# DIVE128/DMVSNet

Measured on AMD Instinct MI355X. Metric: depth-maps/sec, DTU 1600x1184 5-view 3-stage (64/32/8 hyp), higher is better.
Workload: dtype f32; 1 GPU; BASELINE configs[1]: 1600x1184, 5 views, 64/32/8 hypotheses, 3 stage(s) x (main + 4-plane refine); parallelism=1 GPU, k1=warp_corr_q4 (quad-planar features, one launch configuration per shape), conv_backend=auto, streams=2, maps_in_flight=1, hip_graph=False

## Files before the change

### dmvsnet_amd/csrc/conv3d_mfma.hip

```cpp
#ifndef DMVS_KO
#define DMVS_KO 0
#endif
#ifndef DMVS_X
#define DMVS_X 0
#endif
#include "common.h"
#include "tile_loader.h"

#include <algorithm>
#include <cstdlib>
#include <mutex>


#include <map>
#include <type_traits>
#include <utility>

int dmvs_ensure_dynamic_lds(const void* kernel, size_t lds_bytes) {
    static std::mutex mu;
    static std::map<std::pair<int, const void*>, size_t> configured;
    int dev = 0;
    if (hipGetDevice(&dev) != hipSuccess) return (int)hipGetLastError();
    std::lock_guard<std::mutex> lock(mu);
    auto key = std::make_pair(dev, kernel);
    auto it = configured.find(key);
    if (it == configured.end() || it->second < lds_bytes) {
        hipError_t e = hipFuncSetAttribute(kernel, hipFuncAttributeMaxDynamicSharedMemorySize, (int)lds_bytes);
        if (e != hipSuccess) return (int)e;
        configured[key] = lds_bytes;
    }
    return 0;
}

long g_single_buf_min_blocks = 0;
long g_min_blocks = 768, g_split_blocks = 1024;
long g_deconv_prefetch = 1;

#ifdef DMVS_K3_TRACE
__device__ unsigned long long* g_k3_trace;
extern "C" int dmvs_dev_trace_k3(void* p) { return (int)hipMemcpyToSymbol(HIP_SYMBOL(g_k3_trace), &p, sizeof(p)); }
#define K3_NOW() __builtin_amdgcn_s_memtime()
#define K3_TR(slot, val) do { if (threadIdx.x == 0 && g_k3_trace && blockIdx.x < 65536) g_k3_trace[(size_t)blockIdx.x * 16 + (slot)] = (val); } while (0)
#define K3_TR_HW() do { if (threadIdx.x == 0 && g_k3_trace && blockIdx.x < 65536) { unsigned hw, xcc; asm volatile("s_getreg_b32 %0, hwreg(HW_REG_HW_ID)" : "=s"(hw)); \
    asm volatile("s_getreg_b32 %0, hwreg(HW_REG_XCC_ID)" : "=s"(xcc)); g_k3_trace[(size_t)blockIdx.x * 16 + 15] = hw; g_k3_trace[(size_t)blockIdx.x * 16 + 14] = xcc; } } while (0)
#else
#define K3_NOW() 0ull
#define K3_TR(slot, val) do { } while (0)
#define K3_TR_HW() do { } while (0)
#endif

namespace {

struct ConvArgs {
    const float* in;
    float* out;
    const float* w;
    const float* scale;
    const float* shift;
    const float* skip;
    int Cin, Cout, D, H, W, Do, Ho, Wo, relu;
    int skip_up2;
    int nx, ny, nz;
    int st4;
    int in_cs, in_zs, in_elems;
    int single_buf;
    int outq4;
};

typedef float acc16_t __attribute__((ext_vector_type(16)));
typedef float acc4_t __attribute__((ext_vector_type(4)));

template <int M> struct Frag;
template <> struct Frag<32> {
    static constexpr int KK = 2, NV = 32, ACC = 16;
    typedef acc16_t acc_t;
    static __device__ __forceinline__ acc_t mfma(float a, float b, acc_t c) {
        return __builtin_amdgcn_mfma_f32_32x32x2f32(a, b, c, 0, 0, 0);
    }
    static __device__ __forceinline__ int row(int r, int lk) { return (r & 3) + 8 * (r >> 2) + 4 * lk; }
};
template <> struct Frag<16> {
    static constexpr int KK = 4, NV = 16, ACC = 4;
    typedef acc4_t acc_t;
    static __device__ __forceinline__ acc_t mfma(float a, float b, acc_t c) {
        return __builtin_amdgcn_mfma_f32_16x16x4f32(a, b, c, 0, 0, 0);
    }
    static __device__ __forceinline__ int row(int r, int lk) { return lk * 4 + r; }
};

// ... 308 lines not shown
                    : (rok && ox < a.Wo) ? (unsigned)((oz * (a.Ho >> 1) + (oy >> 1)) * (a.Wo >> 1) + (ox >> 1)) * 4u : kInvalid;
                float sk[F::ACC];
#pragma unroll
                for (int rr = 0; rr < F::ACC; ++rr) {
                    const unsigned so = a.skip_up2 ? cooff[rr] >> 2 : cooff[rr];
                    sk[rr] = (DMVS_KO & 4) ? 0.f : __builtin_bit_cast(float, __builtin_amdgcn_raw_buffer_load_b32(rs_skip, ((spos | cooff[rr]) & kInvalid) ? kInvalid : spos + so, 0, 0));
                }
                if (a.outq4) {
                    typedef unsigned v4u_t __attribute__((ext_vector_type(4)));
                    const int ch = a.Cout >> 1, cq = ch >> 2;
#pragma unroll
                    for (int q = 0; q < F::ACC / 4; ++q) {
                        const int co0 = (mb0 + mb) * M + F::row(4 * q, lk), hsel = co0 >= ch ? 1 : 0;
                        float w4[4];
#pragma unroll
                        for (int e = 0; e < 4; ++e) w4[e] = fmaxf(acc[mb][i][xb][4 * q + e] * sc[4 * q + e] + sh[4 * q + e], lo) + sk[4 * q + e];
                        const unsigned off = (!(pos & kInvalid) && co0 < a.Cout)
                            ? (unsigned)(((hsel * a.Do + oz) * cq + ((co0 - hsel * ch) >> 2)) * out_plane + oy * a.Wo + ox) * 16u : kInvalid;
                        v4u_t qv;
                        qv.x = __builtin_bit_cast(unsigned, w4[0]); qv.y = __builtin_bit_cast(unsigned, w4[1]);
                        qv.z = __builtin_bit_cast(unsigned, w4[2]); qv.w = __builtin_bit_cast(unsigned, w4[3]);
                        __builtin_amdgcn_raw_buffer_store_b128(qv, rs_out, off, 0, 0);
                    }
                } else
#pragma unroll
                for (int rr = 0; rr < F::ACC; ++rr) {
                    const unsigned off = (pos | cooff[rr]) & kInvalid ? kInvalid : pos + cooff[rr];
                    const float v = fmaxf(acc[mb][i][xb][rr] * sc[rr] + sh[rr], lo) + sk[rr];
                    if ((DMVS_KO & 4) && v != 1234.56789f) continue;
                    __builtin_amdgcn_raw_buffer_store_b32(__builtin_bit_cast(unsigned, v), rs_out, off, 0, 0);
                }
            }
        }
    }
    }
#ifdef DMVS_K3_TRACE
    asm volatile("s_waitcnt vmcnt(0)" ::: "memory");
    K3_TR(4, K3_NOW());
#endif
}

template <int M, int KD, int CI_CH, int TZ, int TY, bool PYM = false, int NMB = 1>
struct DeconvGeom {
    static constexpr int IZ = KD == 3 ? TZ + 1 : TZ, IY = TY + 1, IX = 33, IXP = 34;
    static constexpr int PS = IZ * IY * IXP;
    static constexpr int GPC = CI_CH / Frag<M>::KK;
    static constexpr int TILE_F = (CI_CH * PS + 63) & ~63;
    static constexpr int WROWS = (PYM ? (KD == 3 ? 18 : 6) : (KD == 3 ? 27 : 9)) * GPC * NMB;
    static constexpr int BUF_F = TILE_F + WROWS * 64;
};

template <int M, int KD, int CI_CH, int TZ, int TY, bool PYM, bool PREF, int NCH = 0, int NMB = 1, bool ZSKIP = false>
__global__ __launch_bounds__(256, (M == 16 ? 3 : 1)) void deconv_mfma_kernel(ConvArgs a) {
    static_assert(!ZSKIP || (KD == 3 && TZ == 1), "the flat tile of a 3x3x3 layer");
    typedef Frag<M> F;
    typedef typename F::acc_t acc_t;
    typedef DeconvGeom<M, KD, CI_CH, TZ, TY, PYM, NMB> G;
    static_assert(NMB == 1 || (NMB == 2 && M == 16 && !PYM && !PREF), "M-block split: two 16-channel blocks");
    static_assert(!PYM || M == 16, "y-parity merge is the Cout = 8 layout of the 16-row MFMA");
    constexpr int NPY = PYM ? 1 : 2;
    constexpr int XB = 32 / F::NV;
    constexpr int NPZ = KD == 3 ? 2 : 1;
    constexpr int IZ = G::IZ, IY = G::IY, IX = G::IX, IXP = G::IXP, PS = G::PS, GPC = G::GPC;
    constexpr int WROWS = G::WROWS, BUF_F = G::BUF_F;
    static_assert(TZ * TY * NMB == 4, "one (input row, M block) per wave");
    extern __shared__ __attribute__((aligned(16))) float smem[];

    const int tid = threadIdx.x, lane = tid & 63;
    const int wave = __builtin_amdgcn_readfirstlane(tid >> 6);
    const int ln = lane % F::NV, lk = lane / F::NV;
    const int rwave = NMB == 2 ? (wave >> 1) : wave, mb = NMB == 2 ? (wave & 1) : 0;
    const int tz = rwave / TY, ty = rwave % TY;
    int bx, by, bz;
    if (!xcd_tile(a.nx, a.ny, a.nz, KD == 3, bx, by, bz)) return;
    const int ix0 = bx * 32, iy0 = by * TY, iz0 = bz * TZ;

    acc_t acc[NPZ][NPY][2][XB];
#pragma unroll
    for (int pz = 0; pz < NPZ; ++pz)
#pragma unroll
        for (int p = 0; p < 2 * NPY; ++p)
#pragma unroll
            for (int xb = 0; xb < XB; ++xb)
#pragma unroll
                for (int r = 0; r < F::ACC; ++r) acc[pz][p >> 1][p & 1][xb][r] = 0.f;

    const int in_vol = a.D * a.H * a.W;
    auto chunk_rsrc = [&](int ci0, int nch) {
        return __builtin_amdgcn_make_buffer_rsrc((void*)(a.in + (size_t)ci0 * in_vol), (short)0, nch * in_vol * 4, 0x00020000);
    };
    const int nchunks = PREF ? NCH : a.Cin / CI_CH;
    const __amdgpu_buffer_rsrc_t rs_w =
        __builtin_amdgcn_make_buffer_rsrc((void*)a.w, (short)0, nchunks * WROWS * 256, 0x00020000);

    constexpr unsigned kInvalid = 0x80000000u;
    constexpr int NGRP = XB * NPZ * NPY;
    const int out_plane = a.Ho * a.Wo, out_vol = a.Do * out_plane;
    const bool has_skip = a.skip != nullptr;
    const char* skp = reinterpret_cast<const char*>(has_skip ? a.skip : a.out);
    float2_t skv[PREF ? NGRP : 1][F::ACC];
    auto group_pos = [&](int g) -> unsigned {
        const int xb = g / (NPZ * NPY), pz = (g / NPY) % NPZ, pyi = g % NPY;
        const int iz = iz0 + tz, iy = iy0 + ty, ix = ix0 + xb * F::NV + ln;
        const bool ok = iz < a.D && iy < a.H && ix < a.W;
        const int py = PYM ? (lk >> 1) : pyi;
        const int oz = KD == 3 ? 2 * iz + pz : iz;
        return ok ? (unsigned)(oz * out_plane + (2 * iy + py) * a.Wo + 2 * ix) * 4u : kInvalid;
    };
    auto chan_off = [&](int rr) -> unsigned {
        const int co = PYM ? (F::row(rr, lk) & 7) : mb * M + F::row(rr, lk);
        return co < a.Cout ? (unsigned)(co * out_vol) * 4u : kInvalid;
    };
    auto prefetch_group = [&](auto g_t) {
        constexpr int g = decltype(g_t)::value;
        if constexpr (PREF) {
            const unsigned pos = group_pos(g);
#pragma unroll
            for (int rr = 0; rr < F::ACC; ++rr) {
                const unsigned co = chan_off(rr);
                const bool inr = !((pos | co) & kInvalid) && has_skip;
                skv[g][rr] = *reinterpret_cast<const float2_t*>(skp + (inr ? (pos + co) : 0u));
            }
        }
    };
    auto prefetch_at = [&](int c) {
        if constexpr (PREF) {
            asm volatile("" ::: "memory");
            static_assert(NGRP <= 8, "prefetch groups");
#define DMVS_PF(G_) if constexpr (G_ < NGRP) { if (c == 0) prefetch_group(std::integral_constant<int, G_>{}); }
            DMVS_PF(0) DMVS_PF(1) DMVS_PF(2) DMVS_PF(3) DMVS_PF(4) DMVS_PF(5) DMVS_PF(6) DMVS_PF(7)
#undef DMVS_PF
            asm volatile("" ::: "memory");
        }
    };

    float sc[F::ACC], sh[F::ACC];
    unsigned cooff[F::ACC];
    auto load_bn = [&]() {
#pragma unroll
    for (int rr = 0; rr < F::ACC; ++rr) {
        const int co = PYM ? (F::row(rr, lk) & 7) : mb * M + F::row(rr, lk);
        const bool cok = co < a.Cout;
        const int coc = cok ? co : 0;
        if (M == 32 && a.Cout == 32 && (DMVS_X & 2)) {
            const int c0 = F::row(rr, 0);
            const float s0 = a.scale ? a.scale[c0] : 1.f, s1 = a.scale ? a.scale[c0 + 4] : 1.f;
            const float h0 = a.scale ? a.shift[c0] : 0.f, h1 = a.scale ? a.shift[c0 + 4] : 0.f;
            sc[rr] = lk ? s1 : s0;
            sh[rr] = lk ? h1 : h0;
        } else {
            sc[rr] = a.scale ? a.scale[coc] : 1.f;
            sh[rr] = a.scale ? a.shift[coc] : 0.f;
        }
        cooff[rr] = cok ? (unsigned)(co * out_vol) * 4u : kInvalid;
    }
    };
    constexpr bool BN_FIRST = PREF || !(DMVS_X & 4);
    if constexpr (BN_FIRST) load_bn();
    if constexpr (PREF) asm volatile("" ::: "memory");
    K3_TR(0, K3_NOW());
    K3_TR_HW();
    [[maybe_unused]] unsigned long long tr_wait = 0, tr_mfma = 0, tr_t = K3_NOW();
    load_tile<CI_CH, IZ, IY, IX, IXP, PS, false>(a.D, a.H, a.W, chunk_rsrc(0, CI_CH), smem, 0, iz0, iy0, ix0, wave, lane);
    load_weights<WROWS>(rs_w, smem + G::TILE_F, 0, wave, lane);
#pragma unroll(PREF ? NCH : 1)
    for (int c = 0; c < (PREF ? NCH : nchunks); ++c) {
        if (PREF && c == 1) {
            static_assert(!PREF || NGRP * F::ACC == 16, "counted wait of the prefetch");
            asm volatile("s_waitcnt vmcnt(16)" ::: "memory");
        } else {
            asm volatile("s_waitcnt vmcnt(0)" ::: "memory");
        }
        __syncthreads();
#ifdef DMVS_K3_TRACE
        { const unsigned long long n = K3_NOW(); tr_wait += n - tr_t; tr_t = n; if (c == 0) K3_TR(1, n); }
#endif
        float* cur = smem + (c & 1) * BUF_F;
        if (c + 1 < nchunks) {
            float* nxt = smem + ((c + 1) & 1) * BUF_F;
            load_tile<CI_CH, IZ, IY, IX, IXP, PS, false>(a.D, a.H, a.W, chunk_rsrc((c + 1) * CI_CH, CI_CH), nxt, (c + 1) * CI_CH, iz0, iy0, ix0, wave, lane);
            load_weights<WROWS>(rs_w, nxt + G::TILE_F, c + 1, wave, lane);
        }
        prefetch_at(c);
        const float* tile = cur;
        const float* wl = cur + G::TILE_F + lane;
        int step = 0;
#pragma unroll
        for (int oz = 0; oz < NPZ; ++oz)
#pragma unroll
            for (int oy = 0; oy < 2; ++oy)
#pragma unroll
                for (int ox = 0; ox < 2; ++ox)
#pragma unroll
                    for (int g = 0; g < GPC; ++g) {
                        if (ZSKIP && oz == 1) continue;
                        float bv[XB];
#pragma unroll
                        for (int xb = 0; xb < XB; ++xb)
                            bv[xb] = tile[(g * F::KK + lk) * PS + ((tz + oz) * IY + ty + oy) * IXP + xb * F::NV + ln + ox];
#pragma unroll
                        for (int pz = oz; pz < NPZ; ++pz)
#pragma unroll
                            for (int py = PYM ? 0 : oy; py < NPY; ++py)
#pragma unroll
                                for (int px = ox; px < 2; ++px) {
                                    const float av = wl[(step * NMB + mb) * 64];
                                    ++step;
#pragma unroll
                                    for (int xb = 0; xb < XB; ++xb)
                                        acc[pz][py][px][xb] = F::mfma(av, bv[xb], acc[pz][py][px][xb]);
                                }
                    }
#ifdef DMVS_K3_TRACE
        { asm volatile("s_nop 0" ::: "memory"); const unsigned long long n = K3_NOW(); tr_mfma += n - tr_t; tr_t = n; }
#endif
    }
    K3_TR(2, K3_NOW());
    K3_TR(8, tr_wait);
    K3_TR(9, tr_mfma);

    typedef unsigned v2u_t __attribute__((ext_vector_type(2)));
    const int iz = iz0 + tz, iy = iy0 + ty;
    const bool rok = iz < a.D && iy < a.H;
    const __amdgpu_buffer_rsrc_t rs_out =
        __builtin_amdgcn_make_buffer_rsrc((void*)a.out, (short)0, a.Cout * out_vol * 4, 0x00020000);
    const float lo = a.relu ? 0.f : -INFINITY;
    if constexpr (!BN_FIRST) load_bn();
#pragma unroll
    for (int xb = 0; xb < XB; ++xb) {
        const int ix = ix0 + xb * F::NV + ln;
        const bool ok = rok && ix < a.W;
#pragma unroll
        for (int pz = 0; pz < NPZ; ++pz)
#pragma unroll
            for (int pyi = 0; pyi < NPY; ++pyi) {
                const int py = PYM ? (lk >> 1) : pyi;
                const int oz = KD == 3 ? 2 * iz + pz : iz;
                const unsigned pos = ok ? (unsigned)(oz * out_plane + (2 * iy + py) * a.Wo + 2 * ix) * 4u : kInvalid;
                float2_t sk[F::ACC];
#pragma unroll
                for (int rr = 0; rr < F::ACC; ++rr) {
                    const bool inr = !((pos | cooff[rr]) & kInvalid) && has_skip;
                    float2_t t;
                    if constexpr (PREF) t = skv[(xb * NPZ + pz) * NPY + pyi][rr];
                    else t = *reinterpret_cast<const float2_t*>(skp + (inr ? (pos + cooff[rr]) : 0u));
                    sk[rr].x = inr ? t.x : 0.f;
                    sk[rr].y = inr ? t.y : 0.f;
                }
#pragma unroll
                for (int rr = 0; rr < F::ACC; ++rr) {
                    const unsigned off = (pos | cooff[rr]) & kInvalid ? kInvalid : pos + cooff[rr];
                    const float vx = fmaxf(acc[pz][pyi][0][xb][rr] * sc[rr] + sh[rr], lo) + sk[rr].x;
                    const float vy = fmaxf(acc[pz][pyi][1][xb][rr] * sc[rr] + sh[rr], lo) + sk[rr].y;
                    v2u_t v;
                    v.x = __builtin_bit_cast(unsigned, vx);
                    v.y = __builtin_bit_cast(unsigned, vy);
                    __builtin_amdgcn_raw_buffer_store_b64(v, rs_out, off, 0, 0);
                }
            }
    }
#ifdef DMVS_K3_TRACE
    K3_TR(3, K3_NOW());
    asm volatile("s_waitcnt vmcnt(0)" ::: "memory");
    K3_TR(4, K3_NOW());
#endif
}

#ifndef DMVS_CONV1_CI
#define DMVS_CONV1_CI 1
#endif
constexpr int CI_CONV1 = DMVS_CONV1_CI;
#include "dev_guard.h"
constexpr int CI_CONV2 = 4, CI_CONV4 = 2, CI_CONV6 = 4, CI_CONV6_2D = 4;
constexpr int CI_F00 = 2, CI_F01 = 4, CI_F1 = 4, CI_F2 = 4, CI_FO3 = 4, CI_K5A = 2, CI_K5B = 2;
constexpr int CI_K1 = 4;
constexpr int DCI11 = 4, DCI9 = 4;
struct Cfg { int cin, cout, mode, kd, M, MB, ci_ch, pym; };
const Cfg kCfgs[] = {
    {2, 16, DMVS_CONV_S1, 3, 16, 1, 2},
    {8, 16, DMVS_CONV_S2, 3, 16, 1, CI_CONV1},
    {16, 16, DMVS_CONV_S1, 3, 16, 1, CI_CONV2},
    {16, 32, DMVS_CONV_S2, 3, 32, 1, 2},
    {32, 32, DMVS_CONV_S1, 3, 32, 1, CI_CONV4},
    {32, 64, DMVS_CONV_S2, 3, 32, 2, 2},
    {64, 64, DMVS_CONV_S1, 3, 32, 2, CI_CONV6},
    {64, 32, DMVS_DECONV_S2, 3, 16, 2, 8},
    {32, 16, DMVS_DECONV_S2, 3, 16, 1, DCI9},
    {16, 8, DMVS_DECONV_S2, 3, 16, 1, DCI11, 1},
    {32, 64, DMVS_CONV_S2, 1, 32, 2, 2},
    {64, 64, DMVS_CONV_S1, 1, 32, 2, CI_CONV6_2D},
    {64, 32, DMVS_DECONV_S2, 1, 16, 2, 8},
    {4, 8, DMVS_CONV_S1, 1, 16, 1, CI_F00},
    {8, 8, DMVS_CONV_S1, 1, 16, 1, CI_F01},
    {8, 16, DMVS_CONV2D_K5S2, 1, 16, 1, CI_K5A},
    {16, 16, DMVS_CONV_S1, 1, 16, 1, CI_F1},
    {16, 32, DMVS_CONV2D_K5S2, 1, 32, 1, CI_K5B},
    {32, 32, DMVS_CONV_S1, 1, 32, 1, CI_F2},
    {32, 16, DMVS_CONV_S1, 1, 16, 1, CI_FO3},
    {32, 64, DMVS_CONV2D_K1, 1, 32, 2, CI_K1},
    {16, 32, DMVS_CONV2D_K1, 1, 32, 1, CI_K1},
    {8, 32, DMVS_CONV2D_K1, 1, 32, 1, CI_K1},
    {16, 32, DMVS_CONV_S1, 1, 32, 1, 4},
    {64, 32, DMVS_CONV2D_K1, 1, 32, 1, CI_K1},
    {32, 16, DMVS_CONV2D_K1, 1, 16, 1, CI_K1},
    {32, 8, DMVS_CONV2D_K1, 1, 16, 1, CI_K1},
};

int taps_of(int mode, int kdepth) {
    return mode == DMVS_CONV2D_K5S2 ? 25 : mode == DMVS_CONV2D_K1 ? 1 : 9 * kdepth;
}

const Cfg* find_cfg(int cin, int cout, int mode, int kdepth) {
    for (const Cfg& c : kCfgs)
        if (c.cin == cin && c.cout == cout && c.mode == mode && c.kd == kdepth) return &c;
    return nullptr;
}

int tap_of(int p, int o) { return p == 0 ? 1 : (o == 0 ? 2 : 0); }
// ... 29 lines not shown

template <int M, int MB, int STRIDE, int KD, int KS, int CI_CH, int TZ, int TY, bool MBS = false>
int launch_conv_tile(const ConvArgs& a, hipStream_t st) {
    return can_v4(a) ? launch_conv_tile_v<M, MB, STRIDE, KD, KS, CI_CH, TZ, TY, true, MBS>(a, st)
                     : launch_conv_tile_v<M, MB, STRIDE, KD, KS, CI_CH, TZ, TY, false, MBS>(a, st);
}

#define kSplitBlocks g_split_blocks
constexpr int kPlanMBS = 1 << 17;
inline int conv_tile_choice(int stride, int kd, int Do, int Ho, int Wo, int MB) {
    const bool flat = (kd == 1) || Do == 1;
    const int big_ty_flat = (stride == 1) ? 16 : 8, big_ty = (stride == 1) ? 8 : 4;
    const long big_blocks = flat ? (long)ceil_div(Wo, 32) * ceil_div(Ho, big_ty_flat) * Do
                                 : (long)ceil_div(Wo, 32) * ceil_div(Ho, big_ty) * ceil_div(Do, 2);
    const bool big = big_blocks >= kMinBlocks;
    if (!big && MB == 2) {
        const long small_blocks = flat ? (long)ceil_div(Wo, 32) * ceil_div(Ho, 4) * Do
                                       : (long)ceil_div(Wo, 32) * ceil_div(Ho, 2) * ceil_div(Do, 2);
        if (small_blocks < kSplitBlocks) return kPlanMBS | (flat ? 256 + 2 : 2 * 256 + 1);
    }
    if (flat) return 256 + (big ? big_ty_flat : 4);
    return 2 * 256 + (big ? big_ty : 2);
}

template <int M, int MB, int STRIDE, int KD, int CI_CH, int KS = 3>
int launch_conv(const ConvArgs& a, hipStream_t st) {
    constexpr int BIG_TY_FLAT = (STRIDE == 1) ? 16 : 8, BIG_TY = (STRIDE == 1) ? 8 : 4;
    const int choice = conv_tile_choice(STRIDE, KD, a.Do, a.Ho, a.Wo, MB);
    const int tz = (choice >> 8) & 255, ty = choice & 255;
    if constexpr (MB == 2) {
        if (choice & kPlanMBS) {
            if (tz == 1) return launch_conv_tile<M, MB, STRIDE, KD, KS, CI_CH, 1, 2, true>(a, st);
            if (KD == 3) return launch_conv_tile<M, MB, STRIDE, 3, 3, CI_CH, 2, 1, true>(a, st);
            return DMVS_EUNSUPPORTED;
        }
    }
    if (tz == 1) {
        if (ty == BIG_TY_FLAT) return launch_conv_tile<M, MB, STRIDE, KD, KS, CI_CH, 1, BIG_TY_FLAT>(a, st);
        return launch_conv_tile<M, MB, STRIDE, KD, KS, CI_CH, 1, 4>(a, st);
    }
    if (KD == 3) {
        if (ty == BIG_TY) return launch_conv_tile<M, MB, STRIDE, 3, 3, CI_CH, 2, BIG_TY>(a, st);
        return launch_conv_tile<M, MB, STRIDE, 3, 3, CI_CH, 2, 2>(a, st);
    }
    return DMVS_EUNSUPPORTED;
}

template <int M, int KD, int CI_CH, int TZ, int TY, bool PYM, int NMB = 1>
int launch_deconv_tile(const ConvArgs& a, hipStream_t st) {
    typedef DeconvGeom<M, KD, CI_CH, TZ, TY, PYM, NMB> G;
    constexpr size_t lds = 2 * (size_t)G::BUF_F * sizeof(float);
    static_assert(lds <= 160 * 1024, "two pipeline stages must fit the 160 KB LDS");
    dim3 grid(ceil_div(a.W, 32), ceil_div(a.H, TY), ceil_div(a.D, TZ));
    const bool zskip = KD == 3 && TZ == 1 && zpad_skip_wanted(a.D) && a.D == 1 && !(zpad_live_mask(DMVS_ZFORM_T2, a.D, 0, 1) & 1u);
    if constexpr (PYM)
        if (a.skip && g_deconv_prefetch && a.Cin == 4 * CI_CH) {
            if constexpr (KD == 3 && TZ == 1)
                if (zskip) return launch_with_lds(deconv_mfma_kernel<M, KD, CI_CH, TZ, TY, PYM, true, 4, 1, true>, grid, lds, a, st);
            return launch_with_lds(deconv_mfma_kernel<M, KD, CI_CH, TZ, TY, PYM, true, 4>, grid, lds, a, st);
        }
    if constexpr (KD == 3 && TZ == 1)
        if (zskip) return launch_with_lds(deconv_mfma_kernel<M, KD, CI_CH, TZ, TY, PYM, false, 0, NMB, true>, grid, lds, a, st);
    return launch_with_lds(deconv_mfma_kernel<M, KD, CI_CH, TZ, TY, PYM, false, 0, NMB>, grid, lds, a, st);
}

template <int M, int KD, int CI_CH, bool PYM = false, int NMB = 1>
int launch_deconv(const ConvArgs& a, hipStream_t st) {
    if constexpr (NMB == 2) {
        if (KD == 1 || a.D == 1) return launch_deconv_tile<M, KD, CI_CH, 1, 2, PYM, 2>(a, st);
        return launch_deconv_tile<M, 3, CI_CH, 2, 1, PYM, 2>(a, st);
    } else {
        if (KD == 1 || a.D == 1) return launch_deconv_tile<M, KD, CI_CH, 1, 4, PYM>(a, st);
        return launch_deconv_tile<M, 3, CI_CH, 2, 2, PYM>(a, st);
    }
}

}

extern "C" long dmvs_conv3d_mfma_weight_floats(int Cin, int Cout, int mode, int kdepth) {
    const Cfg* c = find_cfg(Cin, Cout, mode, kdepth);
    if (!c) return 0;
    const int KK = c->M == 32 ? 2 : 4, nt = taps_of(mode, kdepth);
    if (c->ci_ch < KK) {
        const int tpg = KK / c->ci_ch;
        return (long)(Cin / c->ci_ch) * ((nt + tpg - 1) / tpg) * c->MB * 64;
    }
    if (c->pym) return (long)(nt / 3 * 2) * (Cin / KK) * 64;
    return (long)nt * (Cin / KK) * c->MB * 64;
}

extern "C" int dmvs_pack_conv_weights_mfma(const float* w, float* out, int Cin, int Cout, int mode, int kdepth) {
    const Cfg* c = find_cfg(Cin, Cout, mode, kdepth);
    if (!c || !w || !out) return DMVS_EUNSUPPORTED;
    const int M = c->M, KK = (M == 32 ? 2 : 4), GPC = c->ci_ch / KK, NT = taps_of(mode, kdepth);
    size_t n = 0;
    for (int ci0 = 0; ci0 < Cin; ci0 += c->ci_ch) {
        if (mode != DMVS_DECONV_S2 && c->ci_ch < KK) {
            const int tpg = KK / c->ci_ch, nsteps = (NT + tpg - 1) / tpg;
            for (int st = 0; st < nsteps; ++st)
                for (int mb = 0; mb < c->MB; ++mb)
                    for (int l = 0; l < 64; ++l) {
                        const int co = mb * M + l % M, k = l / M, ci = ci0 + k % c->ci_ch, t = st * tpg + k / c->ci_ch;
                        out[n++] = (co < Cout && t < NT) ? w[((size_t)co * Cin + ci) * NT + t] : 0.f;
                    }
        } else if (mode != DMVS_DECONV_S2) {
            for (int t = 0; t < NT; ++t)
                for (int g = 0; g < GPC; ++g)
                    for (int mb = 0; mb < c->MB; ++mb)
                        for (int l = 0; l < 64; ++l) {
                            const int co = mb * M + l % M, ci = ci0 + g * KK + l / M;
                            out[n++] = co < Cout ? w[((size_t)co * Cin + ci) * NT + t] : 0.f;
                        }
        } else {
            const int npz = kdepth == 3 ? 2 : 1;
            for (int oz = 0; oz < npz; ++oz)
                for (int oy = 0; oy < 2; ++oy)
// ... 101 lines not shown
```

### dmvsnet_amd/csrc/layout.hip

```cpp
#include "common.h"

#include <cstring>

template <int C>
__global__ __launch_bounds__(256) void nchw_to_hwc_kernel(const float* __restrict__ src, long chan_stride, int c0, int HW,
                                                          float* __restrict__ dst) {
    __shared__ float tile[C * 257];
    const int p0 = blockIdx.x * 256;
    const int t = threadIdx.x;
    const int np = min(256, HW - p0);
    if (t < np) {
#pragma unroll
        for (int c = 0; c < C; ++c) tile[c * 257 + t] = src[(size_t)(c0 + c) * chan_stride + p0 + t];
    }
    __syncthreads();
    const int total = np * C;
    float* out = dst + (size_t)p0 * C;
#pragma unroll
    for (int k = 0; k < C; ++k) {
        const int i = k * 256 + t;
        if (i < total) out[i] = tile[(i % C) * 257 + (i / C)];
    }
}

// ... 246 lines not shown
        return;
    }
    float sy = ((float)y + 0.5f) * 0.5f - 0.5f; sy = sy < 0.f ? 0.f : sy;
    float sx = ((float)x + 0.5f) * 0.5f - 0.5f; sx = sx < 0.f ? 0.f : sx;
    const int y0 = (int)sy, x0 = (int)sx;
    const int y1 = min(y0 + 1, h - 1), x1 = min(x0 + 1, w - 1);
    const float ly = sy - (float)y0, lx = sx - (float)x0;
    const float hy = 1.f - ly, hx = 1.f - lx;
    const float l00 = last[y0 * w + x0], l01 = last[y0 * w + x1], l10 = last[y1 * w + x0], l11 = last[y1 * w + x1];
    const bool s00 = ((y0 & 1) == (x0 & 1)), s01 = ((y0 & 1) == (x1 & 1));
    const bool s10 = ((y1 & 1) == (x0 & 1)), s11 = ((y1 & 1) == (x1 & 1));
    for (int d = 0; d < nplanes; ++d) {
        const float v00 = hyp_sample(l00, s00, pix, D, d, inverse), v01 = hyp_sample(l01, s01, pix, D, d, inverse);
        const float v10 = hyp_sample(l10, s10, pix, D, d, inverse), v11 = hyp_sample(l11, s11, pix, D, d, inverse);
        out[((size_t)d * H + y) * W + x] = hy * (hx * v00 + lx * v01) + ly * (hx * v10 + lx * v11);
    }
}

static int hyp_next_launch(const float* last, int h, int w, int up, const float* dv, int n, float ratio, int D, int inverse,
                           float* out, float* out_itv, int nplanes, dmvs_stream_t s) {
    if (!last || !dv || !out || !out_itv || h <= 0 || w <= 0 || n < 2 || D < 2 || (up != 1 && up != 2)) return DMVS_EINVAL;
    dim3 grid(ceil_div(up * w, 256), up * h);
    hyp_next_kernel<<<grid, 256, 0, (hipStream_t)s>>>(last, h, w, dv, n, ratio, D, inverse, out, out_itv, nplanes, up);
    DMVS_LAUNCH_CHECK();
}

extern "C" int dmvs_hypotheses_next(const float* last, int h, int w, const float* dv, int n, float ratio, int D,
                                    int inverse, float* out, float* out_itv, dmvs_stream_t s) {
    return hyp_next_launch(last, h, w, 2, dv, n, ratio, D, inverse, out, out_itv, D, s);
}

extern "C" int dmvs_hypotheses_next_up(const float* last, int h, int w, int up, const float* dv, int n, float ratio, int D,
                                       int inverse, int base_only, float* out, float* out_itv, dmvs_stream_t s) {
    if (base_only && inverse) return DMVS_EINVAL;
    return hyp_next_launch(last, h, w, up, dv, n, ratio, D, inverse, out, out_itv, base_only ? 1 : D, s);
}

extern "C" int dmvs_hypothesis_base_first(const float* dv, int n, int D, int H, int W, float* base_hw, float* out_itv,
                                          dmvs_stream_t s) {
    if (!dv || !base_hw || !out_itv || n < 2 || D < 2 || H <= 0 || W <= 0) return DMVS_EINVAL;
    dim3 grid(ceil_div(W, 256), H, 1);
    hyp_first_kernel<<<grid, 256, 0, (hipStream_t)s>>>(dv, n, D, H, W, 0, base_hw, out_itv);
    DMVS_LAUNCH_CHECK();
}

extern "C" int dmvs_hypothesis_base_next(const float* last, int h, int w, const float* dv, int n, float ratio, int D,
                                         float* base_hw, float* out_itv, dmvs_stream_t s) {
    return hyp_next_launch(last, h, w, 2, dv, n, ratio, D, 0, base_hw, out_itv, 1, s);
}

extern "C" int dmvs_version(void) { return DMVS_VERSION; }

extern long g_single_buf_min_blocks;
extern long g_min_blocks, g_split_blocks, g_wino_stages, g_wino_persistent, g_wino_conv0_grid, g_deconv_prefetch;
extern long g_c8_rows;
extern long g_k3r_grid, g_k3r_counted_wait;
extern long g_k3z_grid, g_k3z_zs;
long g_zpad_skip = 1;

extern "C" long dmvs_zpad_live_mask(int form, int D, int oz0, int TZ) {
    if (form < DMVS_ZFORM_S1 || form > DMVS_ZFORM_T2 || D < 1 || oz0 < 0 || TZ < 1 || TZ > 10) return -1;
    return (long)zpad_live_mask(form, D, oz0, TZ);
}

extern "C" int dmvs_tune(const char* name, int value) {
    if (!name) return DMVS_EINVAL;
    if (!strcmp(name, "k3_single_buf_min_blocks")) { if (value < 0) return DMVS_EINVAL; g_single_buf_min_blocks = value; return 0; }
    if (!strcmp(name, "k3_min_blocks")) { if (value < 0) return DMVS_EINVAL; g_min_blocks = value; return 0; }
    if (!strcmp(name, "k3_split_blocks")) { if (value < 0) return DMVS_EINVAL; g_split_blocks = value; return 0; }
    if (!strcmp(name, "wino_conv0_grid")) { if (value < 8 || value % 8) return DMVS_EINVAL; g_wino_conv0_grid = value; return 0; }
    if (!strcmp(name, "k3_deconv_prefetch")) { g_deconv_prefetch = value ? 1 : 0; return 0; }
    if (!strcmp(name, "c8_rows")) { if (value < 0 || value > 4096) return DMVS_EINVAL; g_c8_rows = value; return 0; }
    if (!strcmp(name, "wino_persistent")) { g_wino_persistent = value ? 1 : 0; return 0; }
    if (!strcmp(name, "k3r_grid")) { if (value < 32 || value > 1024 || value % 32) return DMVS_EINVAL; g_k3r_grid = value; return 0; }
    if (!strcmp(name, "k3z_grid")) { if (value < 0 || value > 4096 || value % 8) return DMVS_EINVAL; g_k3z_grid = value; return 0; }
    if (!strcmp(name, "k3z_zs")) { if (value < 0 || value > 64) return DMVS_EINVAL; g_k3z_zs = value; return 0; }
    if (!strcmp(name, "k3r_counted_wait")) { g_k3r_counted_wait = value ? 1 : 0; return 0; }
    if (!strcmp(name, "zpad_skip")) { if (value != 0 && value != 1) return DMVS_EINVAL; g_zpad_skip = value; return 0; }
    if (!strcmp(name, "wino_stages")) { if (value < 0 || value > 2) return DMVS_EINVAL; g_wino_stages = value; return 0; }
    return DMVS_EUNSUPPORTED;
}

extern "C" const char* dmvs_error_string(int code) {
    if (code == 0) return "ok";
    if (code == DMVS_EINVAL) return "dmvs: invalid argument";
    if (code == DMVS_EUNSUPPORTED) return "dmvs: unsupported channel count or mode";
    if (code > 0) return hipGetErrorString((hipError_t)code);
    return "dmvs: unknown error";
}
```

Baseline: 92.87 depth-maps/s.

## Add quad lane mapping to deconv MFMA kernel for 128-bit output stores

Moves the deconvolution kernel body into a shared include and adds a QUAD variant. In it, each lane owns two adjacent input x positions, reads them with paired float2 LDS loads, and writes four consecutive output x values per channel with one 128-bit buffer store. The skip tensor is also read as float4, so there are fewer, wider global accesses in the epilogue. The variant is enabled by default when W is even and the output and skip pointers are 16-byte aligned, and it changes the LDS access pattern and the counted vmcnt wait of the prefetch path.

Measured after the change: 93.71 depth-maps/s (median of 6 runs). Within noise of the previous version (+0.9%).

```diff
diff --git a/dmvsnet_amd/csrc/conv3d_mfma.hip b/dmvsnet_amd/csrc/conv3d_mfma.hip
--- a/dmvsnet_amd/csrc/conv3d_mfma.hip
+++ b/dmvsnet_amd/csrc/conv3d_mfma.hip
@@ -35,6 +35,7 @@
 long g_single_buf_min_blocks = 0;
 long g_min_blocks = 768, g_split_blocks = 1024;
 long g_deconv_prefetch = 1;
+long g_deconv_quad = 1;
 
 #ifdef DMVS_K3_TRACE
 __device__ unsigned long long* g_k3_trace;
@@ -449,218 +450,14 @@
 
 template <int M, int KD, int CI_CH, int TZ, int TY, bool PYM, bool PREF, int NCH = 0, int NMB = 1, bool ZSKIP = false>
 __global__ __launch_bounds__(256, (M == 16 ? 3 : 1)) void deconv_mfma_kernel(ConvArgs a) {
-    static_assert(!ZSKIP || (KD == 3 && TZ == 1), "the flat tile of a 3x3x3 layer");
-    typedef Frag<M> F;
-    typedef typename F::acc_t acc_t;
-    typedef DeconvGeom<M, KD, CI_CH, TZ, TY, PYM, NMB> G;
-    static_assert(NMB == 1 || (NMB == 2 && M == 16 && !PYM && !PREF), "M-block split: two 16-channel blocks");
-    static_assert(!PYM || M == 16, "y-parity merge is the Cout = 8 layout of the 16-row MFMA");
-    constexpr int NPY = PYM ? 1 : 2;
-    constexpr int XB = 32 / F::NV;
-    constexpr int NPZ = KD == 3 ? 2 : 1;
-    constexpr int IZ = G::IZ, IY = G::IY, IX = G::IX, IXP = G::IXP, PS = G::PS, GPC = G::GPC;
-    constexpr int WROWS = G::WROWS, BUF_F = G::BUF_F;
-    static_assert(TZ * TY * NMB == 4, "one (input row, M block) per wave");
-    extern __shared__ __attribute__((aligned(16))) float smem[];
-
-    const int tid = threadIdx.x, lane = tid & 63;
-    const int wave = __builtin_amdgcn_readfirstlane(tid >> 6);
-    const int ln = lane % F::NV, lk = lane / F::NV;
-    const int rwave = NMB == 2 ? (wave >> 1) : wave, mb = NMB == 2 ? (wave & 1) : 0;
-    const int tz = rwave / TY, ty = rwave % TY;
-    int bx, by, bz;
-    if (!xcd_tile(a.nx, a.ny, a.nz, KD == 3, bx, by, bz)) return;
-    const int ix0 = bx * 32, iy0 = by * TY, iz0 = bz * TZ;
-
-    acc_t acc[NPZ][NPY][2][XB];
-#pragma unroll
-    for (int pz = 0; pz < NPZ; ++pz)
-#pragma unroll
-        for (int p = 0; p < 2 * NPY; ++p)
-#pragma unroll
-            for (int xb = 0; xb < XB; ++xb)
-#pragma unroll
-                for (int r = 0; r < F::ACC; ++r) acc[pz][p >> 1][p & 1][xb][r] = 0.f;
-
-    const int in_vol = a.D * a.H * a.W;
-    auto chunk_rsrc = [&](int ci0, int nch) {
-        return __builtin_amdgcn_make_buffer_rsrc((void*)(a.in + (size_t)ci0 * in_vol), (short)0, nch * in_vol * 4, 0x00020000);
-    };
-    const int nchunks = PREF ? NCH : a.Cin / CI_CH;
-    const __amdgpu_buffer_rsrc_t rs_w =
-        __builtin_amdgcn_make_buffer_rsrc((void*)a.w, (short)0, nchunks * WROWS * 256, 0x00020000);
-
-    constexpr unsigned kInvalid = 0x80000000u;
-    constexpr int NGRP = XB * NPZ * NPY;
-    const int out_plane = a.Ho * a.Wo, out_vol = a.Do * out_plane;
-    const bool has_skip = a.skip != nullptr;
-    const char* skp = reinterpret_cast<const char*>(has_skip ? a.skip : a.out);
-    float2_t skv[PREF ? NGRP : 1][F::ACC];
-    auto group_pos = [&](int g) -> unsigned {
-        const int xb = g / (NPZ * NPY), pz = (g / NPY) % NPZ, pyi = g % NPY;
-        const int iz = iz0 + tz, iy = iy0 + ty, ix = ix0 + xb * F::NV + ln;
-        const bool ok = iz < a.D && iy < a.H && ix < a.W;
-        const int py = PYM ? (lk >> 1) : pyi;
-        const int oz = KD == 3 ? 2 * iz + pz : iz;
-        return ok ? (unsigned)(oz * out_plane + (2 * iy + py) * a.Wo + 2 * ix) * 4u : kInvalid;
-    };
-    auto chan_off = [&](int rr) -> unsigned {
-        const int co = PYM ? (F::row(rr, lk) & 7) : mb * M + F::row(rr, lk);
-        return co < a.Cout ? (unsigned)(co * out_vol) * 4u : kInvalid;
-    };
-    auto prefetch_group = [&](auto g_t) {
-        constexpr int g = decltype(g_t)::value;
-        if constexpr (PREF) {
-            const unsigned pos = group_pos(g);
-#pragma unroll
-            for (int rr = 0; rr < F::ACC; ++rr) {
-                const unsigned co = chan_off(rr);
-                const bool inr = !((pos | co) & kInvalid) && has_skip;
-                skv[g][rr] = *reinterpret_cast<const float2_t*>(skp + (inr ? (pos + co) : 0u));
-            }
-        }
-    };
-    auto prefetch_at = [&](int c) {
-        if constexpr (PREF) {
-            asm volatile("" ::: "memory");
-            static_assert(NGRP <= 8, "prefetch groups");
-#define DMVS_PF(G_) if constexpr (G_ < NGRP) { if (c == 0) prefetch_group(std::integral_constant<int, G_>{}); }
-            DMVS_PF(0) DMVS_PF(1) DMVS_PF(2) DMVS_PF(3) DMVS_PF(4) DMVS_PF(5) DMVS_PF(6) DMVS_PF(7)
-#undef DMVS_PF
-            asm volatile("" ::: "memory");
-        }
-    };
-
-    float sc[F::ACC], sh[F::ACC];
-    unsigned cooff[F::ACC];
-    auto load_bn = [&]() {
-#pragma unroll
-    for (int rr = 0; rr < F::ACC; ++rr) {
-        const int co = PYM ? (F::row(rr, lk) & 7) : mb * M + F::row(rr, lk);
-        const bool cok = co < a.Cout;
-        const int coc = cok ? co : 0;
-        if (M == 32 && a.Cout == 32 && (DMVS_X & 2)) {
-            const int c0 = F::row(rr, 0);
-            const float s0 = a.scale ? a.scale[c0] : 1.f, s1 = a.scale ? a.scale[c0 + 4] : 1.f;
-            const float h0 = a.scale ? a.shift[c0] : 0.f, h1 = a.scale ? a.shift[c0 + 4] : 0.f;
-            sc[rr] = lk ? s1 : s0;
-            sh[rr] = lk ? h1 : h0;
-        } else {
-            sc[rr] = a.scale ? a.scale[coc] : 1.f;
-            sh[rr] = a.scale ? a.shift[coc] : 0.f;
-        }
-        cooff[rr] = cok ? (unsigned)(co * out_vol) * 4u : kInvalid;
-    }
-    };
-    constexpr bool BN_FIRST = PREF || !(DMVS_X & 4);
-    if constexpr (BN_FIRST) load_bn();
-    if constexpr (PREF) asm volatile("" ::: "memory");
-    K3_TR(0, K3_NOW());
-    K3_TR_HW();
-    [[maybe_unused]] unsigned long long tr_wait = 0, tr_mfma = 0, tr_t = K3_NOW();
-    load_tile<CI_CH, IZ, IY, IX, IXP, PS, false>(a.D, a.H, a.W, chunk_rsrc(0, CI_CH), smem, 0, iz0, iy0, ix0, wave, lane);
-    load_weights<WROWS>(rs_w, smem + G::TILE_F, 0, wave, lane);
-#pragma unroll(PREF ? NCH : 1)
-    for (int c = 0; c < (PREF ? NCH : nchunks); ++c) {
-        if (PREF && c == 1) {
-            static_assert(!PREF || NGRP * F::ACC == 16, "counted wait of the prefetch");
-            asm volatile("s_waitcnt vmcnt(16)" ::: "memory");
-        } else {
-            asm volatile("s_waitcnt vmcnt(0)" ::: "memory");
-        }
-        __syncthreads();
-#ifdef DMVS_K3_TRACE
-        { const unsigned long long n = K3_NOW(); tr_wait += n - tr_t; tr_t = n; if (c == 0) K3_TR(1, n); }
-#endif
-        float* cur = smem + (c & 1) * BUF_F;
-        if (c + 1 < nchunks) {
-            float* nxt = smem + ((c + 1) & 1) * BUF_F;
-            load_tile<CI_CH, IZ, IY, IX, IXP, PS, false>(a.D, a.H, a.W, chunk_rsrc((c + 1) * CI_CH, CI_CH), nxt, (c + 1) * CI_CH, iz0, iy0, ix0, wave, lane);
-            load_weights<WROWS>(rs_w, nxt + G::TILE_F, c + 1, wave, lane);
-        }
-        prefetch_at(c);
-        const float* tile = cur;
-        const float* wl = cur + G::TILE_F + lane;
-        int step = 0;
-#pragma unroll
-        for (int oz = 0; oz < NPZ; ++oz)
-#pragma unroll
-            for (int oy = 0; oy < 2; ++oy)
-#pragma unroll
-                for (int ox = 0; ox < 2; ++ox)
-#pragma unroll
-                    for (int g = 0; g < GPC; ++g) {
-                        if (ZSKIP && oz == 1) continue;
-                        float bv[XB];
-#pragma unroll
-                        for (int xb = 0; xb < XB; ++xb)
-                            bv[xb] = tile[(g * F::KK + lk) * PS + ((tz + oz) * IY + ty + oy) * IXP + xb * F::NV + ln + ox];
-#pragma unroll
-                        for (int pz = oz; pz < NPZ; ++pz)
-#pragma unroll
-                            for (int py = PYM ? 0 : oy; py < NPY; ++py)
-#pragma unroll
-                                for (int px = ox; px < 2; ++px) {
-                                    const float av = wl[(step * NMB + mb) * 64];
-                                    ++step;
-#pragma unroll
-                                    for (int xb = 0; xb < XB; ++xb)
-                                        acc[pz][py][px][xb] = F::mfma(av, bv[xb], acc[pz][py][px][xb]);
-                                }
-                    }
-#ifdef DMVS_K3_TRACE
-        { asm volatile("s_nop 0" ::: "memory"); const unsigned long long n = K3_NOW(); tr_mfma += n - tr_t; tr_t = n; }
-#endif
-    }
-    K3_TR(2, K3_NOW());
-    K3_TR(8, tr_wait);
-    K3_TR(9, tr_mfma);
-
-    typedef unsigned v2u_t __attribute__((ext_vector_type(2)));
-    const int iz = iz0 + tz, iy = iy0 + ty;
-    const bool rok = iz < a.D && iy < a.H;
-    const __amdgpu_buffer_rsrc_t rs_out =
-        __builtin_amdgcn_make_buffer_rsrc((void*)a.out, (short)0, a.Cout * out_vol * 4, 0x00020000);
-    const float lo = a.relu ? 0.f : -INFINITY;
-    if constexpr (!BN_FIRST) load_bn();
-#pragma unroll
-    for (int xb = 0; xb < XB; ++xb) {
-        const int ix = ix0 + xb * F::NV + ln;
-        const bool ok = rok && ix < a.W;
-#pragma unroll
-        for (int pz = 0; pz < NPZ; ++pz)
-#pragma unroll
-            for (int pyi = 0; pyi < NPY; ++pyi) {
-                const int py = PYM ? (lk >> 1) : pyi;
-                const int oz = KD == 3 ? 2 * iz + pz : iz;
-                const unsigned pos = ok ? (unsigned)(oz * out_plane + (2 * iy + py) * a.Wo + 2 * ix) * 4u : kInvalid;
-                float2_t sk[F::ACC];
-#pragma unroll
-                for (int rr = 0; rr < F::ACC; ++rr) {
-                    const bool inr = !((pos | cooff[rr]) & kInvalid) && has_skip;
-                    float2_t t;
-                    if constexpr (PREF) t = skv[(xb * NPZ + pz) * NPY + pyi][rr];
-                    else t = *reinterpret_cast<const float2_t*>(skp + (inr ? (pos + cooff[rr]) : 0u));
-                    sk[rr].x = inr ? t.x : 0.f;
-                    sk[rr].y = inr ? t.y : 0.f;
-                }
-#pragma unroll
-                for (int rr = 0; rr < F::ACC; ++rr) {
-                    const unsigned off = (pos | cooff[rr]) & kInvalid ? kInvalid : pos + cooff[rr];
-                    const float vx = fmaxf(acc[pz][pyi][0][xb][rr] * sc[rr] + sh[rr], lo) + sk[rr].x;
-                    const float vy = fmaxf(acc[pz][pyi][1][xb][rr] * sc[rr] + sh[rr], lo) + sk[rr].y;
-                    v2u_t v;
-                    v.x = __builtin_bit_cast(unsigned, vx);
-                    v.y = __builtin_bit_cast(unsigned, vy);
-                    __builtin_amdgcn_raw_buffer_store_b64(v, rs_out, off, 0, 0);
-                }
-            }
-    }
-#ifdef DMVS_K3_TRACE
-    K3_TR(3, K3_NOW());
-    asm volatile("s_waitcnt vmcnt(0)" ::: "memory");
-    K3_TR(4, K3_NOW());
-#endif
+    constexpr bool QUAD = false;
+#include "deconv_mfma_body.inc"
+}
+
+template <int M, int KD, int CI_CH, int TZ, int TY, bool PYM, bool PREF, int NCH = 0, int NMB = 1, bool ZSKIP = false>
+__global__ __launch_bounds__(256, (M == 16 ? 3 : 1)) void deconv_quad_mfma_kernel(ConvArgs a) {
+    constexpr bool QUAD = true;
+#include "deconv_mfma_body.inc"
 }
 
 #ifndef DMVS_CONV1_CI
@@ -796,16 +593,22 @@
     constexpr size_t lds = 2 * (size_t)G::BUF_F * sizeof(float);
     static_assert(lds <= 160 * 1024, "two pipeline stages must fit the 160 KB LDS");
     dim3 grid(ceil_div(a.W, 32), ceil_div(a.H, TY), ceil_div(a.D, TZ));
+    const bool quad = g_deconv_quad && a.W % 2 == 0 && (reinterpret_cast<uintptr_t>(a.out) & 15) == 0 &&
+                      (!a.skip || (reinterpret_cast<uintptr_t>(a.skip) & 15) == 0);
     const bool zskip = KD == 3 && TZ == 1 && zpad_skip_wanted(a.D) && a.D == 1 && !(zpad_live_mask(DMVS_ZFORM_T2, a.D, 0, 1) & 1u);
     if constexpr (PYM)
         if (a.skip && g_deconv_prefetch && a.Cin == 4 * CI_CH) {
             if constexpr (KD == 3 && TZ == 1)
-                if (zskip) return launch_with_lds(deconv_mfma_kernel<M, KD, CI_CH, TZ, TY, PYM, true, 4, 1, true>, grid, lds, a, st);
-            return launch_with_lds(deconv_mfma_kernel<M, KD, CI_CH, TZ, TY, PYM, true, 4>, grid, lds, a, st);
+                if (zskip) return quad ? launch_with_lds(deconv_quad_mfma_kernel<M, KD, CI_CH, TZ, TY, PYM, true, 4, 1, true>, grid, lds, a, st)
+                                       : launch_with_lds(deconv_mfma_kernel<M, KD, CI_CH, TZ, TY, PYM, true, 4, 1, true>, grid, lds, a, st);
+            return quad ? launch_with_lds(deconv_quad_mfma_kernel<M, KD, CI_CH, TZ, TY, PYM, true, 4>, grid, lds, a, st)
+                        : launch_with_lds(deconv_mfma_kernel<M, KD, CI_CH, TZ, TY, PYM, true, 4>, grid, lds, a, st);
         }
     if constexpr (KD == 3 && TZ == 1)
-        if (zskip) return launch_with_lds(deconv_mfma_kernel<M, KD, CI_CH, TZ, TY, PYM, false, 0, NMB, true>, grid, lds, a, st);
-    return launch_with_lds(deconv_mfma_kernel<M, KD, CI_CH, TZ, TY, PYM, false, 0, NMB>, grid, lds, a, st);
+        if (zskip) return quad ? launch_with_lds(deconv_quad_mfma_kernel<M, KD, CI_CH, TZ, TY, PYM, false, 0, NMB, true>, grid, lds, a, st)
+                               : launch_with_lds(deconv_mfma_kernel<M, KD, CI_CH, TZ, TY, PYM, false, 0, NMB, true>, grid, lds, a, st);
+    return quad ? launch_with_lds(deconv_quad_mfma_kernel<M, KD, CI_CH, TZ, TY, PYM, false, 0, NMB>, grid, lds, a, st)
+                : launch_with_lds(deconv_mfma_kernel<M, KD, CI_CH, TZ, TY, PYM, false, 0, NMB>, grid, lds, a, st);
 }
 
 template <int M, int KD, int CI_CH, bool PYM = false, int NMB = 1>
diff --git a/dmvsnet_amd/csrc/deconv_mfma_body.inc b/dmvsnet_amd/csrc/deconv_mfma_body.inc
--- /dev/null
+++ b/dmvsnet_amd/csrc/deconv_mfma_body.inc
@@ -0,0 +1,262 @@
+    static_assert(!ZSKIP || (KD == 3 && TZ == 1), "the flat tile of a 3x3x3 layer");
+    static_assert(!QUAD || M == 16, "the quad mapping pairs the two x blocks of the 16-row MFMA");
+    typedef Frag<M> F;
+    typedef typename F::acc_t acc_t;
+    typedef DeconvGeom<M, KD, CI_CH, TZ, TY, PYM, NMB> G;
+    static_assert(NMB == 1 || (NMB == 2 && M == 16 && !PYM && !PREF), "M-block split: two 16-channel blocks");
+    static_assert(!PYM || M == 16, "y-parity merge is the Cout = 8 layout of the 16-row MFMA");
+    constexpr int NPY = PYM ? 1 : 2;
+    constexpr int XB = 32 / F::NV;
+    constexpr int NPZ = KD == 3 ? 2 : 1;
+    constexpr int IZ = G::IZ, IY = G::IY, IX = G::IX, IXP = G::IXP, PS = G::PS, GPC = G::GPC;
+    constexpr int WROWS = G::WROWS, BUF_F = G::BUF_F;
+    static_assert(TZ * TY * NMB == 4, "one (input row, M block) per wave");
+    extern __shared__ __attribute__((aligned(16))) float smem[];
+
+    const int tid = threadIdx.x, lane = tid & 63;
+    const int wave = __builtin_amdgcn_readfirstlane(tid >> 6);
+    const int ln = lane % F::NV, lk = lane / F::NV;
+    const int rwave = NMB == 2 ? (wave >> 1) : wave, mb = NMB == 2 ? (wave & 1) : 0;
+    const int tz = rwave / TY, ty = rwave % TY;
+    int bx, by, bz;
+    if (!xcd_tile(a.nx, a.ny, a.nz, KD == 3, bx, by, bz)) return;
+    const int ix0 = bx * 32, iy0 = by * TY, iz0 = bz * TZ;
+
+    acc_t acc[NPZ][NPY][2][XB];
+#pragma unroll
+    for (int pz = 0; pz < NPZ; ++pz)
+#pragma unroll
+        for (int p = 0; p < 2 * NPY; ++p)
+#pragma unroll
+            for (int xb = 0; xb < XB; ++xb)
+#pragma unroll
+                for (int r = 0; r < F::ACC; ++r) acc[pz][p >> 1][p & 1][xb][r] = 0.f;
+
+    const int in_vol = a.D * a.H * a.W;
+    auto chunk_rsrc = [&](int ci0, int nch) {
+        return __builtin_amdgcn_make_buffer_rsrc((void*)(a.in + (size_t)ci0 * in_vol), (short)0, nch * in_vol * 4, 0x00020000);
+    };
+    const int nchunks = PREF ? NCH : a.Cin / CI_CH;
+    const __amdgpu_buffer_rsrc_t rs_w =
+        __builtin_amdgcn_make_buffer_rsrc((void*)a.w, (short)0, nchunks * WROWS * 256, 0x00020000);
+
+    constexpr unsigned kInvalid = 0x80000000u;
+    constexpr int NGRP = (QUAD ? 1 : XB) * NPZ * NPY;
+    typedef std::conditional_t<QUAD, float4_t, float2_t> skv_t;
+    const int out_plane = a.Ho * a.Wo, out_vol = a.Do * out_plane;
+    const bool has_skip = a.skip != nullptr;
+    const char* skp = reinterpret_cast<const char*>(has_skip ? a.skip : a.out);
+    skv_t skv[PREF ? NGRP : 1][F::ACC];
+    auto group_pos = [&](int g) -> unsigned {
+        const int xb = g / (NPZ * NPY), pz = (g / NPY) % NPZ, pyi = g % NPY;
+        const int iz = iz0 + tz, iy = iy0 + ty, ix = QUAD ? ix0 + 2 * ln : ix0 + xb * F::NV + ln;
+        const bool ok = iz < a.D && iy < a.H && ix < a.W;
+        const int py = PYM ? (lk >> 1) : pyi;
+        const int oz = KD == 3 ? 2 * iz + pz : iz;
+        return ok ? (unsigned)(oz * out_plane + (2 * iy + py) * a.Wo + 2 * ix) * 4u : kInvalid;
+    };
+    auto chan_off = [&](int rr) -> unsigned {
+        const int co = PYM ? (F::row(rr, lk) & 7) : mb * M + F::row(rr, lk);
+        return co < a.Cout ? (unsigned)(co * out_vol) * 4u : kInvalid;
+    };
+    auto prefetch_group = [&](auto g_t) {
+        constexpr int g = decltype(g_t)::value;
+        if constexpr (PREF) {
+            const unsigned pos = group_pos(g);
+#pragma unroll
+            for (int rr = 0; rr < F::ACC; ++rr) {
+                const unsigned co = chan_off(rr);
+                const bool inr = !((pos | co) & kInvalid) && has_skip;
+                skv[g][rr] = *reinterpret_cast<const skv_t*>(skp + (inr ? (pos + co) : 0u));
+            }
+        }
+    };
+    auto prefetch_at = [&](int c) {
+        if constexpr (PREF) {
+            asm volatile("" ::: "memory");
+            static_assert(NGRP <= 8, "prefetch groups");
+#define DMVS_PF(G_) if constexpr (G_ < NGRP) { if (c == 0) prefetch_group(std::integral_constant<int, G_>{}); }
+            DMVS_PF(0) DMVS_PF(1) DMVS_PF(2) DMVS_PF(3) DMVS_PF(4) DMVS_PF(5) DMVS_PF(6) DMVS_PF(7)
+#undef DMVS_PF
+            asm volatile("" ::: "memory");
+        }
+    };
+
+    float sc[F::ACC], sh[F::ACC];
+    unsigned cooff[F::ACC];
+    auto load_bn = [&]() {
+#pragma unroll
+    for (int rr = 0; rr < F::ACC; ++rr) {
+        const int co = PYM ? (F::row(rr, lk) & 7) : mb * M + F::row(rr, lk);
+        const bool cok = co < a.Cout;
+        const int coc = cok ? co : 0;
+        if (M == 32 && a.Cout == 32 && (DMVS_X & 2)) {
+            const int c0 = F::row(rr, 0);
+            const float s0 = a.scale ? a.scale[c0] : 1.f, s1 = a.scale ? a.scale[c0 + 4] : 1.f;
+            const float h0 = a.scale ? a.shift[c0] : 0.f, h1 = a.scale ? a.shift[c0 + 4] : 0.f;
+            sc[rr] = lk ? s1 : s0;
+            sh[rr] = lk ? h1 : h0;
+        } else {
+            sc[rr] = a.scale ? a.scale[coc] : 1.f;
+            sh[rr] = a.scale ? a.shift[coc] : 0.f;
+        }
+        cooff[rr] = cok ? (unsigned)(co * out_vol) * 4u : kInvalid;
+    }
+    };
+    constexpr bool BN_FIRST = PREF || !(DMVS_X & 4);
+    if constexpr (BN_FIRST) load_bn();
+    if constexpr (PREF) asm volatile("" ::: "memory");
+    K3_TR(0, K3_NOW());
+    K3_TR_HW();
+    [[maybe_unused]] unsigned long long tr_wait = 0, tr_mfma = 0, tr_t = K3_NOW();
+    load_tile<CI_CH, IZ, IY, IX, IXP, PS, false>(a.D, a.H, a.W, chunk_rsrc(0, CI_CH), smem, 0, iz0, iy0, ix0, wave, lane);
+    load_weights<WROWS>(rs_w, smem + G::TILE_F, 0, wave, lane);
+#pragma unroll(PREF ? NCH : 1)
+    for (int c = 0; c < (PREF ? NCH : nchunks); ++c) {
+        if (PREF && c == 1) {
+            static_assert(!PREF || NGRP * F::ACC == (QUAD ? 8 : 16), "counted wait of the prefetch");
+            if constexpr (QUAD) asm volatile("s_waitcnt vmcnt(8)" ::: "memory");
+            else asm volatile("s_waitcnt vmcnt(16)" ::: "memory");
+        } else {
+            asm volatile("s_waitcnt vmcnt(0)" ::: "memory");
+        }
+        __syncthreads();
+#ifdef DMVS_K3_TRACE
+        { const unsigned long long n = K3_NOW(); tr_wait += n - tr_t; tr_t = n; if (c == 0) K3_TR(1, n); }
+#endif
+        float* cur = smem + (c & 1) * BUF_F;
+        if (c + 1 < nchunks) {
+            float* nxt = smem + ((c + 1) & 1) * BUF_F;
+            load_tile<CI_CH, IZ, IY, IX, IXP, PS, false>(a.D, a.H, a.W, chunk_rsrc((c + 1) * CI_CH, CI_CH), nxt, (c + 1) * CI_CH, iz0, iy0, ix0, wave, lane);
+            load_weights<WROWS>(rs_w, nxt + G::TILE_F, c + 1, wave, lane);
+        }
+        prefetch_at(c);
+        const float* tile = cur;
+        const float* wl = cur + G::TILE_F + lane;
+        int step = 0;
+#pragma unroll
+        for (int oz = 0; oz < NPZ; ++oz)
+#pragma unroll
+            for (int oy = 0; oy < 2; ++oy)
+#pragma unroll
+                for (int ox = 0; ox < 2; ++ox)
+#pragma unroll
+                    for (int g = 0; g < GPC; ++g) {
+                        if (ZSKIP && oz == 1) continue;
+                        float bv[XB];
+                        if constexpr (QUAD) {
+                            const float* row = tile + (g * F::KK + lk) * PS + ((tz + oz) * IY + ty + oy) * IXP + 2 * ln;
+                            const float2_t q0 = *reinterpret_cast<const float2_t*>(row), q1 = *reinterpret_cast<const float2_t*>(row + 2);
+                            bv[0] = ox ? q0.y : q0.x;
+                            bv[1] = ox ? q1.x : q0.y;
+                        } else
+#pragma unroll
+                        for (int xb = 0; xb < XB; ++xb)
+                            bv[xb] = tile[(g * F::KK + lk) * PS + ((tz + oz) * IY + ty + oy) * IXP + xb * F::NV + ln + ox];
+#pragma unroll
+                        for (int pz = oz; pz < NPZ; ++pz)
+#pragma unroll
+                            for (int py = PYM ? 0 : oy; py < NPY; ++py)
+#pragma unroll
+                                for (int px = ox; px < 2; ++px) {
+                                    const float av = wl[(step * NMB + mb) * 64];
+                                    ++step;
+#pragma unroll
+                                    for (int xb = 0; xb < XB; ++xb)
+                                        acc[pz][py][px][xb] = F::mfma(av, bv[xb], acc[pz][py][px][xb]);
+                                }
+                    }
+#ifdef DMVS_K3_TRACE
+        { asm volatile("s_nop 0" ::: "memory"); const unsigned long long n = K3_NOW(); tr_mfma += n - tr_t; tr_t = n; }
+#endif
+    }
+    K3_TR(2, K3_NOW());
+    K3_TR(8, tr_wait);
+    K3_TR(9, tr_mfma);
+
+    typedef unsigned v2u_t __attribute__((ext_vector_type(2)));
+    const int iz = iz0 + tz, iy = iy0 + ty;
+    const bool rok = iz < a.D && iy < a.H;
+    const __amdgpu_buffer_rsrc_t rs_out =
+        __builtin_amdgcn_make_buffer_rsrc((void*)a.out, (short)0, a.Cout * out_vol * 4, 0x00020000);
+    const float lo = a.relu ? 0.f : -INFINITY;
+    if constexpr (!BN_FIRST) load_bn();
+    if constexpr (QUAD) {
+        typedef unsigned v4u_t __attribute__((ext_vector_type(4)));
+        constexpr int NG = NPZ * NPY;
+        const bool ok = rok && ix0 + 2 * ln < a.W;
+        auto qpos = [&](int g) -> unsigned {
+            const int pz = g / NPY, py = PYM ? (lk >> 1) : g % NPY;
+            const int oz = KD == 3 ? 2 * iz + pz : iz;
+            return ok ? (unsigned)(oz * out_plane + (2 * iy + py) * a.Wo + 2 * ix0 + 4 * ln) * 4u : kInvalid;
+        };
+        auto load_group = [&](int g, float4_t (&dst)[F::ACC]) {
+            const unsigned pos = qpos(g);
+#pragma unroll
+            for (int rr = 0; rr < F::ACC; ++rr) {
+                const bool inr = !((pos | cooff[rr]) & kInvalid) && has_skip;
+                dst[rr] = *reinterpret_cast<const float4_t*>(skp + (inr ? (pos + cooff[rr]) : 0u));
+            }
+            asm volatile("" ::: "memory");
+        };
+        float4_t ring[2][F::ACC];
+        if constexpr (!PREF) load_group(0, ring[0]);
+#pragma unroll
+        for (int g = 0; g < NG; ++g) {
+            if constexpr (!PREF) { if (g + 1 < NG) load_group(g + 1, ring[(g + 1) & 1]); }
+            const int pz = g / NPY, pyi = g % NPY;
+            const unsigned pos = qpos(g);
+#pragma unroll
+            for (int rr = 0; rr < F::ACC; ++rr) {
+                const bool inr = !((pos | cooff[rr]) & kInvalid) && has_skip;
+                float4_t t;
+                if constexpr (PREF) t = skv[g][rr];
+                else t = ring[g & 1][rr];
+                const unsigned off = (pos | cooff[rr]) & kInvalid ? kInvalid : pos + cooff[rr];
+                v4u_t v;
+                v.x = __builtin_bit_cast(unsigned, fmaxf(acc[pz][pyi][0][0][rr] * sc[rr] + sh[rr], lo) + (inr ? t.x : 0.f));
+                v.y = __builtin_bit_cast(unsigned, fmaxf(acc[pz][pyi][1][0][rr] * sc[rr] + sh[rr], lo) + (inr ? t.y : 0.f));
+                v.z = __builtin_bit_cast(unsigned, fmaxf(acc[pz][pyi][0][1][rr] * sc[rr] + sh[rr], lo) + (inr ? t.z : 0.f));
+                v.w = __builtin_bit_cast(unsigned, fmaxf(acc[pz][pyi][1][1][rr] * sc[rr] + sh[rr], lo) + (inr ? t.w : 0.f));
+                __builtin_amdgcn_raw_buffer_store_b128(v, rs_out, off, 0, 0);
+            }
+        }
+    } else
+#pragma unroll
+    for (int xb = 0; xb < XB; ++xb) {
+        const int ix = ix0 + xb * F::NV + ln;
+        const bool ok = rok && ix < a.W;
+#pragma unroll
+        for (int pz = 0; pz < NPZ; ++pz)
+#pragma unroll
+            for (int pyi = 0; pyi < NPY; ++pyi) {
+                const int py = PYM ? (lk >> 1) : pyi;
+                const int oz = KD == 3 ? 2 * iz + pz : iz;
+                const unsigned pos = ok ? (unsigned)(oz * out_plane + (2 * iy + py) * a.Wo + 2 * ix) * 4u : kInvalid;
+                float2_t sk[F::ACC];
+#pragma unroll
+                for (int rr = 0; rr < F::ACC; ++rr) {
+                    const bool inr = !((pos | cooff[rr]) & kInvalid) && has_skip;
+                    float2_t t;
+                    if constexpr (PREF) t = skv[(xb * NPZ + pz) * NPY + pyi][rr];
+                    else t = *reinterpret_cast<const float2_t*>(skp + (inr ? (pos + cooff[rr]) : 0u));
+                    sk[rr].x = inr ? t.x : 0.f;
+                    sk[rr].y = inr ? t.y : 0.f;
+                }
+#pragma unroll
+                for (int rr = 0; rr < F::ACC; ++rr) {
+                    const unsigned off = (pos | cooff[rr]) & kInvalid ? kInvalid : pos + cooff[rr];
+                    const float vx = fmaxf(acc[pz][pyi][0][xb][rr] * sc[rr] + sh[rr], lo) + sk[rr].x;
+                    const float vy = fmaxf(acc[pz][pyi][1][xb][rr] * sc[rr] + sh[rr], lo) + sk[rr].y;
+                    v2u_t v;
+                    v.x = __builtin_bit_cast(unsigned, vx);
+                    v.y = __builtin_bit_cast(unsigned, vy);
+                    __builtin_amdgcn_raw_buffer_store_b64(v, rs_out, off, 0, 0);
+                }
+            }
+    }
+#ifdef DMVS_K3_TRACE
+    K3_TR(3, K3_NOW());
+    asm volatile("s_waitcnt vmcnt(0)" ::: "memory");
+    K3_TR(4, K3_NOW());
+#endif
diff --git a/dmvsnet_amd/csrc/layout.hip b/dmvsnet_amd/csrc/layout.hip
--- a/dmvsnet_amd/csrc/layout.hip
+++ b/dmvsnet_amd/csrc/layout.hip
@@ -322,7 +322,7 @@
 extern "C" int dmvs_version(void) { return DMVS_VERSION; }
 
 extern long g_single_buf_min_blocks;
-extern long g_min_blocks, g_split_blocks, g_wino_stages, g_wino_persistent, g_wino_conv0_grid, g_deconv_prefetch;
+extern long g_min_blocks, g_split_blocks, g_wino_stages, g_wino_persistent, g_wino_conv0_grid, g_deconv_prefetch, g_deconv_quad;
 extern long g_c8_rows;
 extern long g_k3r_grid, g_k3r_counted_wait;
 extern long g_k3z_grid, g_k3z_zs;
@@ -340,6 +340,7 @@
     if (!strcmp(name, "k3_split_blocks")) { if (value < 0) return DMVS_EINVAL; g_split_blocks = value; return 0; }
     if (!strcmp(name, "wino_conv0_grid")) { if (value < 8 || value % 8) return DMVS_EINVAL; g_wino_conv0_grid = value; return 0; }
     if (!strcmp(name, "k3_deconv_prefetch")) { g_deconv_prefetch = value ? 1 : 0; return 0; }
+    if (!strcmp(name, "k3_deconv_quad")) { if (value != 0 && value != 1) return DMVS_EINVAL; g_deconv_quad = value; return 0; }
     if (!strcmp(name, "c8_rows")) { if (value < 0 || value > 4096) return DMVS_EINVAL; g_c8_rows = value; return 0; }
     if (!strcmp(name, "wino_persistent")) { g_wino_persistent = value ? 1 : 0; return 0; }
     if (!strcmp(name, "k3r_grid")) { if (value < 32 || value > 1024 || value % 32) return DMVS_EINVAL; g_k3r_grid = value; return 0; }
```
